# wangronin/Bayesian-Optimization

Hardware: AMD Instinct MI355X
Metric: candidates/sec (GP posterior+EI) at N=2048,d=20 and ask() wall-time, 1/2/4/8 GPU (higher is better)
Workload: dtype f64

## Files before the change

### bayesian-optimization_amd/_lib.py

```python
from __future__ import annotations

import ctypes as C
import functools
import os
from typing import Optional, Sequence, Tuple

import numpy as np

HERE = os.path.dirname(os.path.abspath(__file__))
LIB_PATH = os.path.join(HERE, "libbogp.so")

OK = 0
ERR_INVALID, ERR_HIP, ERR_NOT_POSDEF, ERR_UNSUPPORTED, ERR_NO_DEVICE, ERR_LLF_POSITIVE = -1, -2, -3, -4, -5, -6
KERNEL_SE, KERNEL_MATERN12, KERNEL_MATERN32, KERNEL_MATERN52, KERNEL_ABSEXP, KERNEL_CUBIC, KERNEL_GENEXP, KERNEL_MATERN_NU = 0, 1, 2, 3, 4, 5, 6, 7
MODE_NOISELESS, MODE_NOISY, MODE_NOISE_ESTIM = 0, 1, 2
ACQ_EI, ACQ_EPSILON_PI, ACQ_UCB, ACQ_MGFI = 0, 1, 2, 3
TREND_CONSTANT, TREND_LINEAR, TREND_QUADRATIC = 0, 1, 2
SELFTEST_PROFILE, SELFTEST_BESSEL_K, SELFTEST_RGAMMA, SELFTEST_BESSEL_K_PAIRS, SELFTEST_MATERN_NU_PAIRS = range(5)
ABI_VERSION = 9
MAX_Q = 64
PRUNE_PATH_NONE, PRUNE_PATH_CHUNKS, PRUNE_PATH_ONEPASS, PRUNE_PATH_ONEPASS_FALLBACK = 0, 1, 2, 3
MAX_TARGETS = 8
MAX_TOPK = 32
MAX_BELIEVED = 32
MAX_PATHS, MAX_FEATURES = 16, 16384
LIFT_MAX_R, LIFT_MAX_RD = 64, 4096
MAX_EHVI_CELLS = 65536
COMM_ID_BYTES = 128
COLUMN_REAL, COLUMN_DISCRETE = 0, 1
SCALES = {"linear": 0, None: 0, "log": 1, "log10": 2, "logit": 3, "bilog": 4}

_dp = C.POINTER(C.c_double)
_ip = C.POINTER(C.c_int)
_lp = C.POINTER(C.c_int64)

SIGNATURES = {
    "bogp_create": (C.c_int, [C.c_int, C.POINTER(C.c_void_p)]),
    "bogp_destroy": (None, [C.c_void_p]),
    "bogp_last_error": (C.c_char_p, [C.c_void_p]),
    "bogp_abi_version": (C.c_int, []),
    "bogp_set_train": (C.c_int, [C.c_void_p, _dp, _dp, C.c_int, C.c_int, C.c_int]),
    "bogp_select_target": (C.c_int, [C.c_void_p, C.c_int]),
    "bogp_nll": (C.c_int, [C.c_void_p, C.c_int, C.c_int, _dp, C.c_int, C.c_double, C.c_int, C.c_int, C.c_double, _dp, _dp]),
    "bogp_nll_batch": (C.c_int, [C.c_void_p, C.c_int, C.c_int, C.c_int, _dp, C.c_int, C.c_double, C.c_int, C.c_int, C.c_double, _dp, _dp, _ip]),
# ... 49 lines not shown
    "bogp_hessian": (C.c_int, [C.c_void_p, _dp, _dp]),
    "bogp_prior_corr": (C.c_int, [C.c_void_p, _dp, C.c_int, _dp]),
    "bogp_point_eval": (C.c_int, [C.c_void_p, _dp, C.c_int, _ip, _dp, C.c_double, C.c_int, _dp, _dp, _dp, _dp, _dp]),
    "bogp_point_eval_batch": (C.c_int, [C.c_void_p, _dp, C.c_int, C.c_int, _ip, _dp, C.c_double, C.c_int, _dp, _dp, _dp, _dp, _dp, _dp]),
    "bogp_polish": (C.c_int, [C.c_void_p, _dp, C.c_int, _dp, _dp, C.c_int, C.c_double, C.c_double, C.c_int, C.c_int, C.c_double,
                              C.c_double, _dp, _dp, _ip]),
    "bogp_point_eval_ehvi": (C.c_int, [C.c_void_p, _dp, C.c_int, C.c_int, C.c_int, _dp, _dp, _dp, _dp, _dp, _dp, _dp, _dp]),
    "bogp_polish_ehvi": (C.c_int, [C.c_void_p, _dp, C.c_int, _dp, _dp, C.c_int, C.c_int, _dp, _dp, C.c_int, C.c_double, C.c_double,
                                   _dp, _dp, _ip]),
    "bogp_comm_unique_id": (C.c_int, [C.c_char_p]),
    "bogp_comm_init": (C.c_int, [C.c_void_p, C.c_char_p, C.c_int, C.c_int]),
    "bogp_comm_attach": (C.c_int, [C.c_void_p, C.c_void_p]),
    "bogp_comm_info": (C.c_int, [C.c_void_p, _ip, _ip]),
    "bogp_comm_destroy": (C.c_int, [C.c_void_p]),
    "bogp_exchange_argmax": (C.c_int, [C.c_void_p, C.c_int64, _dp, _lp, _dp]),
    "bogp_exchange_topk": (C.c_int, [C.c_void_p, C.c_int64, _dp, _lp, _dp]),
    "bogp_reduce_pairs": (C.c_int, [C.c_int, C.c_int, C.c_int, _dp, _dp, _lp, _dp]),
    "bogp_merge_topk": (C.c_int, [C.c_int, C.c_int, C.c_int, C.c_int, _dp, _dp, _lp, _dp]),
    "bogp_last_timing": (C.c_int, [C.c_void_p, _dp, _dp, _dp, _ip]),
    "bogp_set_prune": (C.c_int, [C.c_void_p, C.c_int]),
    "bogp_last_contracted_rows": (C.c_int, [C.c_void_p, _lp]),
    "bogp_last_prune_path": (C.c_int, [C.c_void_p, _ip, _lp, _ip]),
    "bogp_prune_decide": (C.c_int, [C.c_int64, C.c_int64, C.c_int64, C.c_int64]),
    "bogp_sweep_chunk_rows": (C.c_int64, [C.c_int64, C.c_int64, C.c_int64]),
    "bogp_acq_upper_bound": (C.c_double, [C.c_int, C.c_double, C.c_double, C.c_double, C.c_double, C.c_double]),
    "bogp_prune_below": (C.c_int, [C.c_double, C.c_double]),
    "bogp_set_prune_bound32": (C.c_int, [C.c_void_p, C.c_int]),
    "bogp_last_bound32": (C.c_int, [C.c_void_p, _lp, _lp, _ip]),
    "bogp_debug_bound32": (C.c_int, [C.c_void_p, C.c_int64, _dp, _dp, _dp, _dp, C.POINTER(C.c_ubyte), _lp]),
    "bogp_debug_live": (None, [_lp, _lp, _lp]),
    "bogp_bound32_margin": (C.c_int, [C.c_int, C.c_int, C.c_double, C.c_double, C.c_double, C.c_double, _dp, _dp]),
    "bogp_acq_upper_bound_interval": (C.c_double, [C.c_int, C.c_double, C.c_double, C.c_double, C.c_double, C.c_double, C.c_double]),
    "bogp_flops_per_candidate": (C.c_double, [C.c_void_p]),
    "bogp_nll_path": (C.c_int, [C.c_int, C.c_int, C.c_int, C.c_int]),
    "bogp_chol_wide_panels": (C.c_int, [C.c_int, _ip, C.c_int]),
    "bogp_selftest_profile": (C.c_int, [C.c_void_p, C.c_int, C.c_int, C.c_double, _dp, C.c_int64, _dp]),
    "bogp_selftest_gemm": (C.c_int, [C.c_void_p, C.c_int, C.c_int, C.c_int, C.c_int, C.c_int, C.c_double, _dp, C.c_int, _dp, C.c_int, C.c_double, _dp, C.c_int, C.c_int, C.c_int]),
}

_lib = None


class BogpError(RuntimeError):
    def __init__(self, code: int, msg: str):
        super().__init__("libbogp error %d: %s" % (code, msg))
        self.code = code
# ... 888 lines not shown

    def last_bound32(self):
        rows, kept, fb = C.c_int64(), C.c_int64(), C.c_int()
        self._check(self._lib.bogp_last_bound32(self._h, C.cast(C.byref(rows), _lp), C.cast(C.byref(kept), _lp), C.cast(C.byref(fb), _ip)))
        return int(rows.value), int(kept.value), int(fb.value)

    def debug_bound32(self):
        n = C.c_int64()
        self._check(self._lib.bogp_debug_bound32(self._h, 0, None, None, None, None, None, C.cast(C.byref(n), _lp)))
        n = int(n.value)
        out = [np.empty(n) for _ in range(4)]
        flags = np.empty(n, dtype=np.uint8)
        if n:
            m = C.c_int64()
            self._check(self._lib.bogp_debug_bound32(self._h, n, _ptr(out[0]), _ptr(out[1]), _ptr(out[2]), _ptr(out[3]),
                                                     flags.ctypes.data_as(C.POINTER(C.c_ubyte)), C.cast(C.byref(m), _lp)))
        return out[0], out[1], out[2], out[3], flags

    def last_contracted_rows(self) -> int:
        n = C.c_int64()
        self._check(self._lib.bogp_last_contracted_rows(self._h, C.cast(C.byref(n), _lp)))
        return int(n.value)

    def selftest_gemm(self, A, B, C_in=None, ta=False, tb=False, alpha=1.0, beta=0.0, tri=0, split=True):
        A = np.asfortranarray(A, dtype=np.float64)
        B = np.asfortranarray(B, dtype=np.float64)
        m, k = (A.shape[1], A.shape[0]) if ta else A.shape
        k2, n = (B.shape[1], B.shape[0]) if tb else B.shape
        if k != k2:
            raise ValueError("inner dimensions differ: %d vs %d" % (k, k2))
        out = np.zeros((m, n), order="F") if C_in is None else np.asfortranarray(C_in, dtype=np.float64).copy(order="F")
        self._check(self._lib.bogp_selftest_gemm(self._h, int(ta), int(tb), m, n, k, float(alpha), _ptr(A), A.shape[0], _ptr(B), B.shape[0],
                                                 float(beta), _ptr(out), out.shape[0], int(tri), int(split)))
        return out

    def flops_per_candidate(self) -> float:
        return float(self._lib.bogp_flops_per_candidate(self._h))

    def selftest_profile(self, what, arg, kernel=0, pexp=0.0):
        arg = np.ascontiguousarray(arg, dtype=np.float64)
        n = arg.shape[0] if what >= SELFTEST_BESSEL_K_PAIRS else arg.size
        if what >= SELFTEST_BESSEL_K_PAIRS and (arg.ndim != 2 or arg.shape[1] != 2):
            raise ValueError("the *_PAIRS selectors take an (n, 2) array")
        out = np.empty(n)
        self._check(self._lib.bogp_selftest_profile(self._h, int(what), int(kernel), float(pexp), _ptr(arg), n, _ptr(out)))
        return out
# ... 1 lines not shown
```

### bayesian-optimization_amd/csrc/bogp_api.hip

```cpp
#include <hip/hip_runtime.h>

#include <algorithm>
#include <atomic>
#include <cmath>
#include <cstdio>
#include <cstdlib>
#include <cstring>
#include <string>
#include <vector>

#include "../../include/bogp.h"
#include "bogp_handle.h"
#include "bogp_internal.h"
#include "bogp_fit.h"

using namespace bogp;

static std::string g_create_error;

extern "C" int bogp_abi_version(void) { return BOGP_ABI_VERSION; }

extern "C" const char* bogp_last_error(const bogp_handle* h) { return h ? h->err.c_str() : g_create_error.c_str(); }

extern "C" int bogp_create(int device, bogp_handle** out) {
// ... 1 lines not shown
  *out = nullptr;
  int ndev = 0;
  hipError_t e = hipGetDeviceCount(&ndev);
  if (e != hipSuccess || ndev <= 0) {
    g_create_error = std::string("no HIP device: ") + hipGetErrorString(e);
    return BOGP_ERR_NO_DEVICE;
  }
  if (device < 0 || device >= ndev) {
    g_create_error = "device index out of range";
    return BOGP_ERR_INVALID;
  }
  hipDeviceProp_t prop;
  if (hipGetDeviceProperties(&prop, device) != hipSuccess) {
    g_create_error = "hipGetDeviceProperties failed";
    return BOGP_ERR_HIP;
  }
  if (strncmp(prop.gcnArchName, "gfx950", 6) != 0) {
    g_create_error = std::string("libbogp is built for gfx950 only; device is ") + prop.gcnArchName;
    return BOGP_ERR_NO_DEVICE;
  }
  bogp_handle* h = new bogp_handle();
  h->device = device;
  h->n_cu = prop.multiProcessorCount > 0 ? prop.multiProcessorCount : 256;
  int prio_least = 0, prio_greatest = 0;
  if (hipSetDevice(device) != hipSuccess || hipDeviceGetStreamPriorityRange(&prio_least, &prio_greatest) != hipSuccess ||
      hipStreamCreateWithPriority(&h->stream, hipStreamNonBlocking, prio_greatest) != hipSuccess ||
      hipStreamCreateWithPriority(&h->stream2, hipStreamNonBlocking, prio_least) != hipSuccess ||
      h->dscal.ensure(h, 64) != BOGP_OK) {
    g_create_error = "stream creation failed";
    delete h;
    return BOGP_ERR_HIP;
  }
  if (h->hfit.ensure(h, 4096) != BOGP_OK) {
    g_create_error = "pinned host buffer allocation failed";
    delete h;
    return BOGP_ERR_HIP;
  }
  h->hfit_dev = h->hfit.dev;
  if (h->dfin_ticket.ensure(h, 1) != BOGP_OK || hipMemset(h->dfin_ticket, 0, sizeof(unsigned int)) != hipSuccess) {
    g_create_error = "device allocation failed";
    delete h;
    return BOGP_ERR_HIP;
  }
  h->dinfo = reinterpret_cast<int*>(h->dscal + 62);
  if (!h->ev_chol.at(1)) {
    g_create_error = "event creation failed";
// ... 245 lines not shown
```

### bayesian-optimization_amd/csrc/bogp_api_sweep.hip

```cpp
#include <hip/hip_runtime.h>

#include <algorithm>
#include <atomic>
#include <cmath>
#include <cstdio>
#include <cstdlib>
#include <cstring>
#include <string>
#include <vector>

#include "../../include/bogp.h"
#include "bogp_device.h"
#include "bogp_handle.h"
#include "bogp_internal.h"
#include "bogp_fit.h"

using namespace bogp;

void bogp::invalidate_sweep_results(bogp_handle* h) { h->last_q = h->last_topk_q = h->last_topk_k = 0; }

static int lazy_copy_to(bogp_handle* h, int64_t upto) {
  if (!h->hXs_lazy) return BOGP_OK;
  upto = std::min<int64_t>(upto, h->M);
  if (upto <= h->lazy_done) return BOGP_OK;
// ... 542 lines not shown
      aa.uu = h->duu;
    }
  }
  aa.mtrend = h->dmtrend;
  aa.estimate_trend = 0;
  return BOGP_OK;
}

static int sweep_pruned_chunk(bogp_handle* h, SweepCtx& cx, const AcqArgs& model, const ContractArgs& ka, int64_t c, int64_t c_end, int64_t m0, int64_t mcount, int64_t skip) {
  hipStream_t st = cx.st;
  long long* const pctl = cx.pctl;
  const int64_t Mc = cx.g.Mc, Ms = cx.Ms, nblk_total = cx.nblk_total;
  const int q = cx.rq.q;
  hipEvent_t* ev = &h->ev[(size_t)(c * EPC)];
  int64_t i0 = 0;
  if (skip > 0) i0 = skip;
  else if (c == 0) {
    const int64_t P = std::min<int64_t>(PRUNE_PILOT, mcount);
    hipEvent_t* evp = &h->ev[(size_t)(cx.g.nchunk * EPC + 1)];
    HIPCHK(h, launch_prune_init(pctl, h->dbest_val, h->dbest_idx, q, P, st));
    HIPCHK(h, hipEventRecord(evp[0], st));
    ContractArgs kp = ka;
    kp.nMt = (int)((P + 63) / 64);
    HIPCHK(h, launch_contract(kp, st));
    HIPCHK(h, hipEventRecord(evp[1], st));
    AcqArgs ap = model;
    ap.mu_part = h->dmu_part[0]; ap.w_part = h->dw_part[0]; ap.ss_part = h->dss_part; ap.Mc = Mc; ap.mcount = P; ap.m0 = 0;
    HIPCHK(h, launch_acquisition(ap, st));
    HIPCHK(h, launch_prune_update(h->dblk_val, h->dblk_idx, nblk_total, nullptr, P, q, h->dbest_val, h->dbest_idx, st));
    i0 = P;
  }
  const int64_t rcount = mcount - i0;
  if (rcount > 0) {
    PruneBoundArgs pb = prune_bound_args(h, cx);
    pb.mu_part = h->dmu_part[0] + i0; pb.w_part = h->dw_part[0] + i0; pb.Mc = Mc; pb.rcount = rcount;
    HIPCHK(h, launch_prune_bound(pb, st));
    HIPCHK(h, launch_prune_scan(cx.pblk_count, (rcount + 255) / 256, cx.poffsets, rcount, Ms, pctl, st));
    PruneGatherArgs pg;
    pg.ctl = pctl; pg.flags = cx.pflags; pg.offsets = cx.poffsets; pg.rcount = rcount; pg.m0 = m0 + i0; pg.Mc = Mc; pg.Ms = Ms; pg.S = cx.g.S;
    pg.Np = h->Np; pg.rT = h->drT[0] + i0; pg.mu_part = h->dmu_part[0] + i0; pg.w_part = h->dw_part[0] + i0;
    pg.rTs = h->drT[1]; pg.mu_s = h->dmu_part[1]; pg.w_s = h->dw_part[1]; pg.sel = cx.psel; pg.map = cx.pmap;
    HIPCHK(h, launch_prune_gather(pg, st));
    cx.prune_pending += rcount / 4;
  }
  const bool flush = cx.prune_pending > 0 && (c + 1 == c_end || cx.prune_pending + Mc / 4 > Ms);
  HIPCHK(h, hipEventRecord(ev[2], st));
  if (rcount > 0) {
    ContractArgs ki = ka;
    ki.rT = h->drT[0] + i0; ki.ss_part = h->dss_part + i0; ki.nMt = (int)((rcount + 63) / 64); ki.live = pctl + 1;
    HIPCHK(h, launch_contract(ki, st));
  }
  if (flush) {
    ContractArgs kf = ka;
    kf.rT = h->drT[1]; kf.ss_part = cx.dss_surv; kf.Mc = Ms; kf.nMt = (int)(Ms / 64); kf.live = pctl + 0;
    HIPCHK(h, launch_contract(kf, st));
  }
  HIPCHK(h, hipEventRecord(ev[3], st));
  if (rcount > 0) {
    AcqArgs ai = model;
    ai.mu_part = h->dmu_part[0] + i0; ai.w_part = h->dw_part[0] + i0; ai.ss_part = h->dss_part + i0; ai.Mc = Mc; ai.mcount = rcount;
    ai.m0 = m0 + i0; ai.live = pctl + 1;
    HIPCHK(h, launch_acquisition(ai, st));
    HIPCHK(h, launch_prune_update(h->dblk_val, h->dblk_idx, nblk_total, pctl + 1, 0, q, h->dbest_val, h->dbest_idx, st));
  }
  if (flush) {
    AcqArgs af = model;
    af.mu_part = h->dmu_part[1]; af.w_part = h->dw_part[1]; af.ss_part = cx.dss_surv; af.Mc = Ms; af.mcount = Ms; af.m0 = 0;
    af.live = pctl + 0; af.map = cx.pmap;
    HIPCHK(h, launch_acquisition(af, st));
    HIPCHK(h, launch_prune_update(h->dblk_val, h->dblk_idx, nblk_total, pctl + 0, 0, q, h->dbest_val, h->dbest_idx, st));
    HIPCHK(h, launch_prune_flushed(pctl, st));
    cx.prune_pending = 0;
  }
  HIPCHK(h, hipEventRecord(ev[4], st));
  return BOGP_OK;
}

static int sweep_chunks(bogp_handle* h, SweepCtx& cx, int64_t c_begin, int64_t c_end, bool pilot_done) {
// ... 17 lines not shown
    ka.rT = h->drT[b]; ka.Vp = vx ? h->dVpx : h->dVp; ka.ss_part = h->dss_part; ka.Mc = Mc; ka.nMt = (int)(Mc_eff / 64); ka.nJ = cx.nJ;
    ka.NJ16 = cx.NJ16; ka.NKP = cx.Nrows / 8;
    if (overlap && c >= 2) HIPCHK(h, hipStreamWaitEvent(stP, h->ev[(size_t)((c - 2) * EPC + 4)], 0));
    if (overlap && vx && c >= 1) HIPCHK(h, hipStreamWaitEvent(stP, h->ev[(size_t)((c - 1) * EPC + 4)], 0));
    int e;
    if ((e = lazy_copy_to(h, m0 + mcount)) || (e = lazy_wait(h, stP)) || (stP != st && (e = lazy_wait(h, st)))) return e;
    HIPCHK(h, hipEventRecord(ev[0], stP));
    const int64_t skip = pilot_done && c == 0 ? std::min<int64_t>(PRUNE_PILOT, mcount) : 0;
    if (skip > 0) {
      ca.m0 += skip; ca.rT += skip; ca.mu_part += skip; ca.w_part += skip;
    }
    if (Mc_eff > skip) HIPCHK(h, launch_corr_chunk(h->kernel, ca, (int)((Mc_eff - skip) / 64), S, stP));
    if (vx) {
      if (h->vx_Ne > Np) HIPCHK(h, hipMemsetAsync(h->drT[b] + (size_t)Np * Mc, 0, (size_t)(h->vx_Ne - Np) * Mc * sizeof(double), stP));
      HIPCHK(h, launch_trend_rows(h->trend, h->dXs, m0, mcount, Mc_eff, h->d, Mc, h->dbetav, h->drT[b] + (size_t)h->vx_Ne * Mc, h->p,
                                  h->vx_Nt - h->vx_Ne, h->dmtrend, stP));
    }
    HIPCHK(h, hipEventRecord(ev[1], stP));
    if (overlap) HIPCHK(h, hipStreamWaitEvent(st, ev[1], 0));
    if (cx.prune) {
      if ((e = sweep_pruned_chunk(h, cx, model, ka, c, c_end, m0, mcount, skip))) return e;
    } else {
      HIPCHK(h, hipEventRecord(ev[2], st));
      if (rq.need_var) HIPCHK(h, launch_contract(ka, st));
      HIPCHK(h, hipEventRecord(ev[3], st));
      AcqArgs aa = model;
      aa.mu_part = h->dmu_part[b]; aa.w_part = h->dw_part[b]; aa.ss_part = h->dss_part; aa.nJ = rq.need_var ? cx.nJ_main : 0; aa.Mc = Mc;
      aa.nJ_plus = vx ? cx.nJ - cx.nJ_main : 0;
      aa.mcount = mcount; aa.m0 = m0; aa.blk_offset = cx.blk_offset;
      if (h->p > 1 && (e = sweep_trend_chunk(h, cx, b, m0, mcount, Mc_eff, aa))) return e;
      if (rq.eh) {
        EhviArgs ea = *rq.eh;
        ea.rT = h->drT[b]; ea.ss_part = h->dss_part; ea.w_part = h->dw_part[b]; ea.S = S; ea.nJ = cx.nJ_main; ea.Mc = Mc;
        ea.mcount = mcount; ea.m0 = m0; ea.beta = h->beta; ea.G = h->G; ea.estimate_trend = h->estimate_trend;
        ea.ehvi_out = h->dacq_out; ea.mu_out = rq.want_out ? h->dmu_out : nullptr; ea.mse_out = rq.want_out ? h->dmse_out : nullptr;
        ea.blk_val = h->dblk_val; ea.blk_idx = h->dblk_idx; ea.blk_offset = cx.blk_offset;
        HIPCHK(h, launch_ehvi(ea, st));
      } else {
        HIPCHK(h, launch_acquisition(aa, st));
      }
      HIPCHK(h, hipEventRecord(ev[4], st));
    }
    cx.blk_offset += (mcount + 255) / 256;
    if ((e = lazy_copy_to(h, m0 + mcount + Mc))) return e;
  }
  return BOGP_OK;
}
// ... 23 lines not shown
  const int64_t P = std::min<int64_t>(PRUNE_PILOT, Mc);
  long long* const hcount = reinterpret_cast<long long*>(h->hfit + 3504);
  size_t ev_next = (size_t)(nchunk * EPC + 3);
  h->t_spans.clear(); h->t_chunks.clear();
  int e;
  auto survivors_of = [&](int64_t rows, int64_t index_from, long long* out, const unsigned char* flags, int64_t* sidx, const int64_t* through) -> int {
    HIPCHK(h, launch_prune_scan(cx.pblk_count, (rows + 255) / 256, cx.poffsets, rows, -1, pctl, st));
    if (index_from >= 0) HIPCHK(h, launch_prune_index(flags, cx.poffsets, rows, index_from, cx.sidx_cap, sidx, st, through));
    HIPCHK(h, hipMemcpyAsync(hcount, pctl + PRUNE_CTL_TOTAL, sizeof(long long), hipMemcpyDeviceToHost, st));
    HIPCHK(h, hipStreamSynchronize(st));
    *out = *hcount;
    return BOGP_OK;
  };
  const CorrArgs cc = corr_chunk_args(h, cx.g, 0, 1);
  ContractArgs kc;
  kc.rT = h->drT[1]; kc.Vp = h->dVp; kc.ss_part = cx.dss_surv; kc.Mc = Ms; kc.nJ = cx.nJ; kc.NJ16 = cx.NJ16; kc.NKP = cx.Nrows / 8;
  AcqArgs aa = acq_model_args(h, cx.rq, S, cx.nJ_main, nblk_total);
  aa.mu_part = h->dmu_part[1]; aa.w_part = h->dw_part[1]; aa.ss_part = cx.dss_surv; aa.Mc = Ms; aa.m0 = 0;
  PruneBoundArgs pb = prune_bound_args(h, cx);
  Bound32Model md32{h->dX32, h->dvec32, h->dvec32 + h->Np, h->dvec32 + 2 * (size_t)h->Np, h->stats32[0], h->stats32[1], h->stats32[2]};
  int contract_launches = 0;
  auto evaluate = [&](int64_t cnt, const int64_t* map) -> int {
    kc.nMt = (int)((cnt + 63) / 64);
    if (int e2 = timed_span(h, st, &ev_next, 1, [&] { return launch_contract(kc, st); })) return e2;
    ++contract_launches;
    aa.mcount = cnt; aa.map = map;
    HIPCHK(h, launch_acquisition(aa, st));
    HIPCHK(h, launch_prune_update(h->dblk_val, h->dblk_idx, nblk_total, nullptr, cnt, q, h->dbest_val, h->dbest_idx, st));
    return BOGP_OK;
  };
  auto fall_back = [&](int64_t c0, int64_t c1, int path) -> int {
    int e2;
    if ((e2 = h->drT[0].ensure(h, (size_t)cx.Nrows * Mc))) return e2;
    if ((e2 = sweep_chunks(h, cx, c0, c1, true))) return e2;
    for (int64_t c = c0; c < c1; ++c) h->t_chunks.push_back(c);
    contract_launches += (int)(c1 - c0);
    h->prune_path = path;
    return BOGP_OK;
  };
  if ((e = mark_event(h, st, &ev_next, &h->t_total[0]))) return e;
  HIPCHK(h, launch_prune_init(pctl, h->dbest_val, h->dbest_idx, q, P, st));
  if ((e = timed_span(h, st, &ev_next, 0, [&] { return launch_corr_chunk(kernel, cc, (int)(P / 64), S, st); }))) return e;
  if ((e = evaluate(P, nullptr))) return e;
  long long pilot_surv = 0;
  pb.mu_part = h->dmu_part[1]; pb.w_part = h->dw_part[1]; pb.Mc = Ms; pb.rcount = P;
  HIPCHK(h, launch_prune_bound(pb, st));
  if ((e = survivors_of(P, -1, &pilot_surv, cx.pflags, cx.psidx, nullptr))) return e;
// ... 270 lines not shown
  if (rounds) *rounds = h->prune_rounds;
  return BOGP_OK;
}

extern "C" int bogp_prune_decide(int64_t pilot_rows, int64_t pilot_survivors, int64_t segment_rows, int64_t segment_survivors) {
  return prune_decide(pilot_rows, pilot_survivors, segment_rows, segment_survivors);
}
extern "C" int64_t bogp_sweep_chunk_rows(int64_t rows, int64_t M, int64_t chunk_bytes) { return sweep_chunk_rows(rows, M, chunk_bytes); }

extern "C" int bogp_last_contracted_rows(bogp_handle* h, int64_t* rows) {
  if (!h) return BOGP_ERR_INVALID;
  if (!rows) FAIL(h, BOGP_ERR_INVALID, "bogp_last_contracted_rows: null output");
  *rows = h->contracted_rows;
  if (h->prune_used && h->dprune) {
    HIPCHK(h, hipSetDevice(h->device));
    long long n = 0;
    HIPCHK(h, hipMemcpyAsync(&n, h->dprune + PRUNE_CTL_CONTRACTED, sizeof(n), hipMemcpyDeviceToHost, h->stream));
    HIPCHK(h, hipStreamSynchronize(h->stream));
    *rows = (int64_t)n + h->prune_survivors;
  }
  return BOGP_OK;
}

extern "C" double bogp_acq_upper_bound(int acq_id, double acq_par, double y_hat, double sd_ub, double plugin, double sigma2) {
  return acq_upper_bound(acq_id, acq_par, y_hat, sd_ub, plugin, sigma2);
}
extern "C" int bogp_prune_below(double bound, double threshold) { return prune_below(bound, threshold) ? 1 : 0; }

extern "C" double bogp_flops_per_candidate(const bogp_handle* h) {
  if (!h || !h->committed) return 0.0;
  const double N = h->N, d = h->d, p = h->estimate_trend ? 1 : 0;
  return N * N + N * (3 * d + 5 + 2 * p);
}

extern "C" int bogp_gradient(bogp_handle* h, const double* x, double* dmu, double* dmse) {
  if (!h) return BOGP_ERR_INVALID;
  if (!h->committed) FAIL(h, BOGP_ERR_INVALID, "bogp_gradient: no committed model");
  if (h->kernel == BOGP_KERNEL_CUBIC || h->kernel == BOGP_KERNEL_GENEXP || h->kernel == BOGP_KERNEL_MATERN_NU) FAIL(h, BOGP_ERR_UNSUPPORTED, "bogp_gradient: the cubic correlation has no input-derivative (corr_dx leaves it undefined in the reference, gpr.py:655-658)");
  if (!x || !dmu || !dmse) FAIL(h, BOGP_ERR_INVALID, "bogp_gradient: null pointer");
  const int N = h->N, d = h->d;
  hipStream_t st = h->stream;
  HIPCHK(h, hipSetDevice(h->device));
  const int pt = h->p;
  if (pt == 1)
    return point_eval_host(h, "bogp_gradient", x, 1, 0, nullptr, nullptr, 0.0, 1, nullptr, nullptr, dmu, dmse, nullptr, nullptr);
  if (pt > 1 && h->trend == BOGP_TREND_QUADRATIC)
// ... 139 lines not shown
```

### bayesian-optimization_amd/csrc/bogp_handle.h

```cpp
#pragma once
#include <hip/hip_runtime.h>

#include <atomic>
#include <cstdio>
#include <cstring>
#include <string>
#include <vector>

#include "../../include/bogp.h"
#include "bogp_internal.h"

struct bogp_handle;
namespace bogp {
void comm_release(bogp_handle* h);
std::vector<bogp_handle*> nll_team(bogp_handle* h, int P);
int point_eval_host(bogp_handle* h, const char* who, const double* Xb, int B, int q, const int* acq_id, const double* acq_par,
                    double plugin, int minimize, double* mu, double* mse, double* dmu, double* dmse, double* acq, double* dacq);
struct SweepRequest {
  bool want_out = false, want_acq_out = false;
  bool need_var = true, sync = true;
  int q = 0, minimize = 1;
  const int* acq_id = nullptr;
  const double* acq_par = nullptr;
  double plugin = 0.0;
// ... 113 lines not shown
  int kernel = 0, mode = 0, estimate_trend = 0;
  double beta = 0, G = 0, sigma2 = 0, noise_var = 0, llf = 0, ftft = 0;
  bogp::DevBuf<double> dXthT;
  bogp::DevBuf<double> dXnorm;
  bogp::DevBuf<double2> dVpx;
  bogp::DevBuf<double> dAtx;
  int vx_Ne = 0, vx_Nt = 0;
  bogp::DevBuf<double2> dVp;

  const double* dXs = nullptr;
  bogp::DevBuf<double> dXs_owned;
  bogp::DevBuf<double> dbounds;
  bogp::DevBuf<double> dxform;
  std::vector<double> h_xform;
  bogp::DevBuf<double> dsobol;
  int64_t M = 0;
  const double* hXs_lazy = nullptr;
  int64_t lazy_done = 0;
  hipStream_t stream_copy = nullptr;
  bogp::EventPool ev_copy{hipEventDisableTiming};

  bogp::DevBuf<double> drT[2], dmu_part[2], dw_part[2];
  bogp::DevBuf<double> dss_part;
  bogp::DevBuf<double> dblk_val, dmu_out, dmse_out, dacq_out, dbest_val;
  bogp::DevBuf<int64_t> dblk_idx, dbest_idx;
  bogp::DevBuf<unsigned int> dcounter;
  int prune_mode = 1;
  int prune_path = 0;
  int64_t prune_survivors = 0;
  int prune_rounds = 0;
  bogp::DevBuf<long long> dprune;
  int prune_bound32 = 1;
  bogp::DevBuf<float> dX32, dvec32;
  bogp::DevBuf<double> dstats32;
  double stats32[3] = {0, 0, 0};
  uint64_t commit_gen = 0, b32_gen = 0;
  int b32_target = -1;
  int64_t b32_rows = 0, b32_kept = 0;
  int b32_fallbacks = 0;
  size_t b32_ws_row32 = 0, b32_ws_flag1 = 0, b32_ws_rmax = 0;
  int64_t b32_last_rows = 0;
  bool prune_used = false;
  int64_t contracted_rows = 0;
  bogp::DevBuf<double> dtopk_val;
  bogp::DevBuf<int64_t> dtopk_idx;
  bogp::DevBuf<double> dehvi_cells;
// ... 148 lines not shown
```

### bayesian-optimization_amd/csrc/bogp_internal.h

```cpp
#pragma once
#include <hip/hip_runtime.h>
#include <stdint.h>

#include <string>

#include "../../include/bogp.h"

namespace bogp {

struct CorrArgs {
  const double* Xs;
  int64_t M;
  int64_t m0;
  int64_t Mc;
  int d;
  int Np;
  int nblk_per_split;
  const double* sqrt_theta;
  const double* XthT;
  const double* xnorm = nullptr;
  const double* gamma;
  const double* wvec;
  double* rT;
  bool store = true;
// ... 7 lines not shown
inline int train_ld(int N) { return N > 3072 ? ((N + 127) / 128) * 128 : ((N + 63) / 64) * 64; }
constexpr int SWEEP_NBLK_PER_SPLIT = 8;
inline int sweep_slices(int Np) { return (Np / 32 + SWEEP_NBLK_PER_SPLIT - 1) / SWEEP_NBLK_PER_SPLIT; }
constexpr int64_t SWEEP_MAX_CHUNK_ROWS = ((((int64_t)1 << 29) - 31) / 7) / 64 * 64;
inline int64_t sweep_chunk_rows(int64_t rows, int64_t M, int64_t chunk_bytes) {
  const int64_t Mpad = (M + 63) / 64 * 64, fit = chunk_bytes / (rows * (int64_t)sizeof(double)) / 64 * 64;
  const int64_t Mc = fit < 64 ? 64 : fit < Mpad ? fit : Mpad;
  return Mc > SWEEP_MAX_CHUNK_ROWS ? -1 : Mc;
}
int corr_trend_columns(int p);
bool corr_chunk_without_store(int kernel, int pv, bool have_xnorm);

struct ContractArgs {
  const double* rT;
  const double2* Vp;
  double* ss_part;
  int64_t Mc;
  int nMt;
  int nJ;
  int NJ16;
  int NKP;
  int64_t cross_B;
  const long long* live = nullptr;
};

struct AcqArgs {
  const double* mu_part;
  const double* w_part;
  const double* ss_part;
  int S, nJ;
  int nJ_plus = 0;
  int64_t Mc;
  int64_t mcount;
  int64_t m0;
  double beta;
  const double* mtrend;
  const double* uu;
  double G;
  int estimate_trend;
  double sigma2;
  double* mu_out;
  double* mse_out;
  int q;
  int acq_id[64];
  double acq_par[64];
  double plugin;
// ... 249 lines not shown
  double beta, G, sigma2, plugin;
  int estimate_trend, minimize, q;
  int acq_id[64];
  double acq_par[64];
  double* mu_out;
  double* mse_out;
  double* acq_out;
  double* blk_val;
  int64_t* blk_idx;
  int64_t nblk;
  unsigned int* counter;
  double* best_val;
  int64_t* best_idx;
  long long* stamps;
  int64_t m_begin;
  int64_t blk_begin;
  int final_launch;
};
bool sweep_small_supported(int Np, int d, int kernel);
int64_t sweep_small_blocks(int64_t M, int n_cu);
hipError_t launch_sweep_small(int kernel, const SmallArgs& a, int n_cu, hipStream_t st);

hipError_t launch_corr_chunk(int kernel, const CorrArgs& a, int nMt, int S, hipStream_t st);
hipError_t launch_contract(const ContractArgs& a, hipStream_t st);
hipError_t launch_contract_cross(const ContractArgs& a, int ncp, hipStream_t st);
int contract_cols_per_group();
hipError_t launch_acquisition(const AcqArgs& a, hipStream_t st);
hipError_t launch_argmax_final(const double* blk_val, const int64_t* blk_idx, int64_t nblk, int64_t stride, int q,
                               double* out_val, int64_t* out_idx, hipStream_t st);

hipError_t launch_topk(const double* vals, int64_t M, int q, int k, double* blk_val, int64_t* blk_idx, double* out_val,
                       int64_t* out_idx, hipStream_t st);

struct LiftArgs {
  const double* Z;
  int64_t M;
  int r, D;
  const double* lift;
  double* penalty;
  int* blk_count;
};
size_t lift_lds_bytes(int r, int D);
hipError_t launch_lift_penalty(const LiftArgs& a, hipStream_t st);
hipError_t launch_lift_scan(const int* blk_count, int64_t nblk, int64_t* offsets, hipStream_t st);
hipError_t launch_lift_compact(const double* Z, int64_t M, int r, const double* penalty, const int64_t* offsets, double* Zc,
                               int64_t* map, hipStream_t st);
hipError_t launch_lift_merge(const double* penalty, int64_t M, const double* acq, const int64_t* map, int64_t Mf, int q,
// ... 236 lines not shown
```

### bayesian-optimization_amd/csrc/kernels_posterior.hip

```cpp
#include <algorithm>
#include <cstdlib>

#include "bogp_device.h"
#include "bogp_internal.h"
#include "bogp_mfma.h"

namespace bogp {

struct CorrDims {
  int64_t M, m0, Mc;
  int d, Np, nblk_per_split;
  int wld;
};
template <int KERNEL, int PV>
__global__ __launch_bounds__(256) void k_corr_chunk(const double* __restrict__ Xs, const double* __restrict__ sqrt_theta,
                                                    const double* __restrict__ XthT, const double* __restrict__ gamma,
                                                    const double* __restrict__ wvec, double* __restrict__ rT,
                                                    double* __restrict__ mu_part, double* __restrict__ w_part,
                                                    const double* __restrict__ Wrow, double* __restrict__ t_part, CorrDims a) {
  extern __shared__ __attribute__((aligned(16))) double smem[];
  double* xs = smem;
  const int tid = threadIdx.x;
  const int m = tid & 63;
  const int g = __builtin_amdgcn_readfirstlane(tid >> 6);
// ... 87 lines not shown
                                                   CorrDims a) {
#define BOGP_CORR_STORE 1
#include "corr_mfma_body.inc"
#undef BOGP_CORR_STORE
}
template <int KERNEL>
__global__ __launch_bounds__(256) __attribute__((amdgpu_waves_per_eu(4, 4))) void k_corr_mfma_sums(const double* __restrict__ Xs, const double* __restrict__ sqrt_theta,
                                                   const double* __restrict__ XthT, const double* __restrict__ xnorm,
                                                   const double* __restrict__ gamma, const double* __restrict__ wvec,
                                                   double* __restrict__ mu_part, double* __restrict__ w_part, CorrDims a) {
#define BOGP_CORR_STORE 0
#include "corr_mfma_body.inc"
#undef BOGP_CORR_STORE
}

#undef BOGP_OPQ
constexpr int MR = 4;
constexpr int NWJ = 4;
constexpr int KB = 32;
constexpr int PITCH = 64 + 16;



template <int NR>
__device__ __forceinline__ void contract_drain(d4 (&acc)[MR][NR]) {
#ifndef BOGP_LINT_NO_DRAIN
  mfma16_drain();
#endif
#ifndef BOGP_LINT_NO_FENCE
#pragma unroll
  for (int mi = 0; mi < MR; ++mi)
#pragma unroll
    for (int ni = 0; ni < NR; ++ni) mfma16_fence(acc[mi][ni]);
#endif
}

template <int NR, bool GUARDED>
__device__ __forceinline__ void contract_block16(const double* __restrict__ tile, const double2* __restrict__ vp,
                                                 const size_t (&boff)[NR], const int (&jt)[NR], int aoff, int kb, int kp_last,
                                                 double2 (&bq)[4][NR], d4 (&acc)[MR][NR]) {
  double af[2][MR];
#pragma unroll
  for (int mi = 0; mi < MR; ++mi) af[0][mi] = tile[aoff + 16 * mi];
#pragma unroll
  for (int s = 0; s < 4; ++s) {
    const int kp = kb * 4 + s;
    const int kb16 = kp >> 1;
    {
      const int kpn = min(kp + 2, kp_last);
#pragma unroll
      for (int ni = 0; ni < NR; ++ni) bq[(s + 2) & 3][ni] = vp[boff[ni] + (size_t)kpn * 64];
    }
#pragma unroll
    for (int h = 0; h < 2; ++h) {
// ... 322 lines not shown
    red2[w * 64 + lane] = s;
  }
  BOGP_DT_NOW(5);
  __syncthreads();
  if (tid < 64) {
    const double tot = ((red2[tid] + red2[64 + tid]) + red2[128 + tid]) + red2[192 + tid];
    a.ss_part[(size_t)jg * a.Mc + mc0 + tid] = tot;
  }
#ifdef CONTRACT_D_TRACE
  BOGP_DT_NOW(6);
  dtr[7] = (unsigned long long)nkp | ((unsigned long long)nkp_full << 32);
  __syncthreads();
  if (trace_out) {
    unsigned long long* dst = trace_out + (size_t)blockIdx.x * (NWJ * DT_NST);
    const unsigned long long* src = &dtr_all[0][0];
    for (int i = tid; i < NWJ * DT_NST; i += 256) dst[i] = src[i];
  }
#endif
}
#undef BOGP_DT_NOW
#undef BOGP_DT_ISSUE
#undef BOGP_DT_STORE

static bool corr_sqdist_kernel(int kernel) {
  return kernel == BOGP_KERNEL_SE || kernel == BOGP_KERNEL_MATERN12 || kernel == BOGP_KERNEL_MATERN32 || kernel == BOGP_KERNEL_MATERN52;
}
bool corr_chunk_without_store(int kernel, int pv, bool have_xnorm) { return corr_sqdist_kernel(kernel) && pv == 0 && have_xnorm; }

hipError_t launch_corr_chunk(int kernel, const CorrArgs& a, int nMt, int S, hipStream_t st) {
  dim3 grid((unsigned)nMt, (unsigned)S);
  if (corr_chunk_without_store(kernel, a.pv, a.xnorm != nullptr)) {
    const int KS = (a.d + 3) / 4;
    const size_t shm = (size_t)max(4 * KS * 64, 2048) * sizeof(double);
    CorrDims dm{a.M, a.m0, a.Mc, a.d, a.Np, a.nblk_per_split, a.wld};
#define BOGP_LAUNCH_CORR_MFMA(K)                                                                                                      \
  do {                                                                                                                                \
    if (shm > 64 * 1024) {                                                                                                            \
      hipError_t e_ = hipFuncSetAttribute(reinterpret_cast<const void*>(&k_corr_mfma<K>), hipFuncAttributeMaxDynamicSharedMemorySize, \
                                          (int)shm);                                                                                  \
      if (e_ != hipSuccess) return e_;                                                                                                \
    }                                                                                                                                 \
    hipLaunchKernelGGL((k_corr_mfma<K>), grid, 256, shm, st, a.Xs, a.sqrt_theta, a.XthT, a.xnorm, a.gamma, a.wvec, a.rT, a.mu_part,   \
                       a.w_part, dm);                                                                                                 \
  } while (0)
#define BOGP_LAUNCH_CORR_SUMS(K)                                                                                                      \
  do {                                                                                                                                \
// ... 63 lines not shown

#ifdef CONTRACT_D_TRACE
static unsigned long long* g_trace = nullptr;
static size_t g_trace_words = 0, g_trace_used = 0;
static int g_trace_dims[4] = {0, 0, 0, 0};
hipError_t debug_contract_trace(unsigned long long* out, size_t cap_words, size_t* used_words, int* dims) {
  if (used_words) *used_words = g_trace_used;
  if (dims) for (int i = 0; i < 4; ++i) dims[i] = g_trace_dims[i];
  if (!out) return hipSuccess;
  hipError_t e = hipDeviceSynchronize();
  if (e != hipSuccess) return e;
  return hipMemcpy(out, g_trace, std::min(cap_words, g_trace_used) * sizeof(unsigned long long), hipMemcpyDeviceToHost);
}
#else
static bool contract_direct() {
  static const bool on = [] {
    const char* e = getenv("BOGP_CONTRACT_DIRECT");
    return !(e && atoi(e) == 0);
  }();
  return on;
}
#endif

hipError_t launch_contract(const ContractArgs& a, hipStream_t st) {
  const dim3 grid((unsigned)(a.nMt * a.nJ));
#ifdef CONTRACT_D_TRACE
  const size_t need = (size_t)a.nMt * a.nJ * NWJ * DT_NST;
  if (need > g_trace_words) {
    if (g_trace) (void)hipFree(g_trace);
    hipError_t e = hipMalloc((void**)&g_trace, need * sizeof(unsigned long long));
    if (e != hipSuccess) return e;
    g_trace_words = need;
  }
  const bool keep = need >= g_trace_used;
  if (keep) {
    g_trace_used = need;
    g_trace_dims[0] = a.nMt; g_trace_dims[1] = a.nJ; g_trace_dims[2] = a.NJ16; g_trace_dims[3] = DT_NST;
  }
  hipLaunchKernelGGL(k_contract16d, grid, 256, 0, st, a, keep ? g_trace : (unsigned long long*)nullptr);
#else
  if (contract_direct()) hipLaunchKernelGGL(k_contract16d, grid, 256, 0, st, a);
  else hipLaunchKernelGGL(k_contract16<4>, grid, 256, 0, st, a);
#endif
  return hipGetLastError();
}

int contract_cols_per_group() { return NWJ * 4 * 16; }

hipError_t launch_contract_cross(const ContractArgs& a, int ncp, hipStream_t st) {
  const dim3 grid((unsigned)(a.nMt * a.nJ));
  if (ncp == 16) hipLaunchKernelGGL((k_contract16<4, 16>), grid, 256, 0, st, a);
  else if (ncp == 32) hipLaunchKernelGGL((k_contract16<4, 32>), grid, 256, 0, st, a);
  else if (ncp == 64) hipLaunchKernelGGL((k_contract16<4, 64>), grid, 256, 0, st, a);
  else return hipErrorInvalidValue;
  return hipGetLastError();
}

}
```

### include/bogp.h

```cpp
#ifndef BOGP_H
#define BOGP_H

#include <stdint.h>

#ifdef __cplusplus
extern "C" {
#endif

typedef struct bogp_handle bogp_handle;

#define BOGP_ABI_VERSION 9
#define BOGP_OK 0
#define BOGP_ERR_INVALID (-1)
#define BOGP_ERR_HIP (-2)
#define BOGP_ERR_NOT_POSDEF (-3)
#define BOGP_ERR_UNSUPPORTED (-4)
#define BOGP_ERR_NO_DEVICE (-5)
#define BOGP_ERR_LLF_POSITIVE (-6)

#define BOGP_KERNEL_SE 0
#define BOGP_KERNEL_MATERN12 1
#define BOGP_KERNEL_MATERN32 2
#define BOGP_KERNEL_MATERN52 3
#define BOGP_KERNEL_ABSEXP 4
// ... 156 lines not shown
int bogp_comm_info(const bogp_handle* h, int* rank, int* world);
int bogp_comm_destroy(bogp_handle* h);
int bogp_exchange_argmax(bogp_handle* h, int64_t index_offset, double* best_val, int64_t* best_gidx, double* best_x);
int bogp_exchange_topk(bogp_handle* h, int64_t index_offset, double* best_val, int64_t* best_gidx, double* best_x);
int bogp_reduce_pairs(int R, int q, int d, const double* gathered, double* val, int64_t* gidx, double* x);
int bogp_merge_topk(int R, int q, int k, int d, const double* gathered, double* val, int64_t* gidx, double* x);

int bogp_last_timing(bogp_handle* h, double* corr_ms, double* contract_ms, double* acquisition_ms, int* n_chunks);

int bogp_set_prune(bogp_handle* h, int on);

#define BOGP_PRUNE_PATH_NONE 0
#define BOGP_PRUNE_PATH_CHUNKS 1
#define BOGP_PRUNE_PATH_ONEPASS 2
#define BOGP_PRUNE_PATH_ONEPASS_FALLBACK 3
int bogp_last_prune_path(bogp_handle* h, int* path, int64_t* survivors, int* rounds);

int bogp_prune_decide(int64_t pilot_rows, int64_t pilot_survivors, int64_t segment_rows, int64_t segment_survivors);

int64_t bogp_sweep_chunk_rows(int64_t rows, int64_t M, int64_t chunk_bytes);

int bogp_last_contracted_rows(bogp_handle* h, int64_t* rows);

double bogp_acq_upper_bound(int acq_id, double acq_par, double y_hat, double sd_ub, double plugin, double sigma2);
int bogp_prune_below(double bound, double threshold);

int bogp_set_prune_bound32(bogp_handle* h, int on);

int bogp_last_bound32(bogp_handle* h, int64_t* rows, int64_t* kept, int* fallbacks);

int bogp_debug_bound32(bogp_handle* h, int64_t cap, double* mu32, double* e_mu, double* wd32, double* e_w, unsigned char* flags, int64_t* rows);

void bogp_debug_live(int64_t* allocations, int64_t* bytes, int64_t* events);

int bogp_bound32_margin(int kernel, int d, double na, double nb_max, double gamma_l1, double w_l1, double* e_mu, double* e_w);
double bogp_acq_upper_bound_interval(int acq_id, double acq_par, double y_hat, double e, double sd_ub, double plugin, double sigma2);

double bogp_flops_per_candidate(const bogp_handle* h);

int bogp_selftest_gemm(bogp_handle* h, int ta, int tb, int m, int n, int k, double alpha, const double* A, int lda,
                       const double* B, int ldb, double beta, double* C, int ldc, int tri, int split);

#define BOGP_SELFTEST_PROFILE 0
#define BOGP_SELFTEST_BESSEL_K 1
#define BOGP_SELFTEST_RGAMMA 2
#define BOGP_SELFTEST_BESSEL_K_PAIRS 3
// ... 19 lines not shown
```

Measured before the change: 531.8 million.

## Add smaller-row contract kernels chosen by occupancy heuristic for small candidate batches

```diff
diff --git a/bayesian-optimization_amd/_lib.py b/bayesian-optimization_amd/_lib.py
--- a/bayesian-optimization_amd/_lib.py
+++ b/bayesian-optimization_amd/_lib.py
@@ -20,6 +20,7 @@
 ABI_VERSION = 9
 MAX_Q = 64
 PRUNE_PATH_NONE, PRUNE_PATH_CHUNKS, PRUNE_PATH_ONEPASS, PRUNE_PATH_ONEPASS_FALLBACK = 0, 1, 2, 3
+CONTRACT_TILE64_MIN_WG_PER_4CU, CONTRACT_TILE32_MIN_WG_PER_4CU = 14, 6
 MAX_TARGETS = 8
 MAX_TOPK = 32
 MAX_BELIEVED = 32
@@ -115,6 +116,9 @@
     "bogp_last_contracted_rows": (C.c_int, [C.c_void_p, _lp]),
     "bogp_last_prune_path": (C.c_int, [C.c_void_p, _ip, _lp, _ip]),
     "bogp_prune_decide": (C.c_int, [C.c_int64, C.c_int64, C.c_int64, C.c_int64]),
+    "bogp_set_contract_tile": (C.c_int, [C.c_void_p, C.c_int]),
+    "bogp_last_contract_tile": (C.c_int, [C.c_void_p, _ip]),
+    "bogp_contract_tile_rows": (C.c_int, [C.c_int64, C.c_int, C.c_int, C.c_int]),
     "bogp_sweep_chunk_rows": (C.c_int64, [C.c_int64, C.c_int64, C.c_int64]),
     "bogp_acq_upper_bound": (C.c_double, [C.c_int, C.c_double, C.c_double, C.c_double, C.c_double, C.c_double]),
     "bogp_prune_below": (C.c_int, [C.c_double, C.c_double]),
@@ -1049,6 +1053,16 @@
         self._check(self._lib.bogp_last_contracted_rows(self._h, C.cast(C.byref(n), _lp)))
         return int(n.value)
 
+    def set_contract_tile(self, rows=0):
+        if rows not in (0, 16, 32, 64):
+            raise ValueError("set_contract_tile: %r is none of 0 (automatic), 16, 32, 64" % (rows,))
+        self._check(self._lib.bogp_set_contract_tile(self._h, int(rows)))
+
+    def last_contract_tile(self) -> int:
+        n = C.c_int()
+        self._check(self._lib.bogp_last_contract_tile(self._h, C.cast(C.byref(n), _ip)))
+        return int(n.value)
+
     def selftest_gemm(self, A, B, C_in=None, ta=False, tb=False, alpha=1.0, beta=0.0, tri=0, split=True):
         A = np.asfortranarray(A, dtype=np.float64)
         B = np.asfortranarray(B, dtype=np.float64)
diff --git a/bayesian-optimization_amd/csrc/bogp_api.hip b/bayesian-optimization_amd/csrc/bogp_api.hip
--- a/bayesian-optimization_amd/csrc/bogp_api.hip
+++ b/bayesian-optimization_amd/csrc/bogp_api.hip
@@ -47,6 +47,7 @@
   bogp_handle* h = new bogp_handle();
   h->device = device;
   h->n_cu = prop.multiProcessorCount > 0 ? prop.multiProcessorCount : 256;
+  h->contract_tile.n_cu = h->n_cu;
   int prio_least = 0, prio_greatest = 0;
   if (hipSetDevice(device) != hipSuccess || hipDeviceGetStreamPriorityRange(&prio_least, &prio_greatest) != hipSuccess ||
       hipStreamCreateWithPriority(&h->stream, hipStreamNonBlocking, prio_greatest) != hipSuccess ||
diff --git a/bayesian-optimization_amd/csrc/bogp_api_sweep.hip b/bayesian-optimization_amd/csrc/bogp_api_sweep.hip
--- a/bayesian-optimization_amd/csrc/bogp_api_sweep.hip
+++ b/bayesian-optimization_amd/csrc/bogp_api_sweep.hip
@@ -588,7 +588,7 @@
     HIPCHK(h, hipEventRecord(evp[0], st));
     ContractArgs kp = ka;
     kp.nMt = (int)((P + 63) / 64);
-    HIPCHK(h, launch_contract(kp, st));
+    HIPCHK(h, launch_contract(kp, st, h->contract_tile));
     HIPCHK(h, hipEventRecord(evp[1], st));
     AcqArgs ap = model;
     ap.mu_part = h->dmu_part[0]; ap.w_part = h->dw_part[0]; ap.ss_part = h->dss_part; ap.Mc = Mc; ap.mcount = P; ap.m0 = 0;
@@ -614,12 +614,12 @@
   if (rcount > 0) {
     ContractArgs ki = ka;
     ki.rT = h->drT[0] + i0; ki.ss_part = h->dss_part + i0; ki.nMt = (int)((rcount + 63) / 64); ki.live = pctl + 1;
-    HIPCHK(h, launch_contract(ki, st));
+    HIPCHK(h, launch_contract(ki, st, h->contract_tile));
   }
   if (flush) {
     ContractArgs kf = ka;
     kf.rT = h->drT[1]; kf.ss_part = cx.dss_surv; kf.Mc = Ms; kf.nMt = (int)(Ms / 64); kf.live = pctl + 0;
-    HIPCHK(h, launch_contract(kf, st));
+    HIPCHK(h, launch_contract(kf, st, h->contract_tile));
   }
   HIPCHK(h, hipEventRecord(ev[3], st));
   if (rcount > 0) {
@@ -683,7 +683,7 @@
       if ((e = sweep_pruned_chunk(h, cx, model, ka, c, c_end, m0, mcount, skip))) return e;
     } else {
       HIPCHK(h, hipEventRecord(ev[2], st));
-      if (rq.need_var) HIPCHK(h, launch_contract(ka, st));
+      if (rq.need_var) HIPCHK(h, launch_contract(ka, st, h->contract_tile));
       HIPCHK(h, hipEventRecord(ev[3], st));
       AcqArgs aa = model;
       aa.mu_part = h->dmu_part[b]; aa.w_part = h->dw_part[b]; aa.ss_part = h->dss_part; aa.nJ = rq.need_var ? cx.nJ_main : 0; aa.Mc = Mc;
@@ -753,7 +753,7 @@
   int contract_launches = 0;
   auto evaluate = [&](int64_t cnt, const int64_t* map) -> int {
     kc.nMt = (int)((cnt + 63) / 64);
-    if (int e2 = timed_span(h, st, &ev_next, 1, [&] { return launch_contract(kc, st); })) return e2;
+    if (int e2 = timed_span(h, st, &ev_next, 1, [&] { return launch_contract(kc, st, h->contract_tile); })) return e2;
     ++contract_launches;
     aa.mcount = cnt; aa.map = map;
     HIPCHK(h, launch_acquisition(aa, st));
@@ -1070,6 +1070,20 @@
   return BOGP_OK;
 }
 
+extern "C" int bogp_set_contract_tile(bogp_handle* h, int rows) {
+  if (!h) return BOGP_ERR_INVALID;
+  if (rows != 0 && rows != 16 && rows != 32 && rows != 64) FAIL(h, BOGP_ERR_INVALID, "bogp_set_contract_tile: %d is none of 0 (automatic), 16, 32, 64", rows);
+  h->contract_tile.forced = rows;
+  return BOGP_OK;
+}
+extern "C" int bogp_last_contract_tile(bogp_handle* h, int* rows) {
+  if (!h) return BOGP_ERR_INVALID;
+  if (!rows) FAIL(h, BOGP_ERR_INVALID, "bogp_last_contract_tile: null output");
+  *rows = h->contract_tile.last;
+  return BOGP_OK;
+}
+extern "C" int bogp_contract_tile_rows(int64_t row_tiles64, int nJ, int n_cu, int live) { return contract_tile_rows(row_tiles64, nJ, n_cu, live != 0); }
+
 extern "C" double bogp_acq_upper_bound(int acq_id, double acq_par, double y_hat, double sd_ub, double plugin, double sigma2) {
   return acq_upper_bound(acq_id, acq_par, y_hat, sd_ub, plugin, sigma2);
 }
diff --git a/bayesian-optimization_amd/csrc/bogp_handle.h b/bayesian-optimization_amd/csrc/bogp_handle.h
--- a/bayesian-optimization_amd/csrc/bogp_handle.h
+++ b/bayesian-optimization_amd/csrc/bogp_handle.h
@@ -159,6 +159,7 @@
 
   bogp::DevBuf<double> drT[2], dmu_part[2], dw_part[2];
   bogp::DevBuf<double> dss_part;
+  bogp::ContractTile contract_tile;
   bogp::DevBuf<double> dblk_val, dmu_out, dmse_out, dacq_out, dbest_val;
   bogp::DevBuf<int64_t> dblk_idx, dbest_idx;
   bogp::DevBuf<unsigned int> dcounter;
diff --git a/bayesian-optimization_amd/csrc/bogp_internal.h b/bayesian-optimization_amd/csrc/bogp_internal.h
--- a/bayesian-optimization_amd/csrc/bogp_internal.h
+++ b/bayesian-optimization_amd/csrc/bogp_internal.h
@@ -53,6 +53,21 @@
   int NKP;
   int64_t cross_B;
   const long long* live = nullptr;
+};
+
+constexpr int CONTRACT_TILE64_MIN_WG_PER_4CU = 14;
+constexpr int CONTRACT_TILE32_MIN_WG_PER_4CU = 6;
+inline int contract_tile_rows(int64_t tiles64, int nJ, int n_cu, bool live) {
+  if (live) return 64;
+  const int64_t wg4 = 4 * tiles64 * (int64_t)(nJ > 0 ? nJ : 1), cu = n_cu > 0 ? n_cu : 1;
+  if (wg4 >= CONTRACT_TILE64_MIN_WG_PER_4CU * cu) return 64;
+  if (wg4 >= CONTRACT_TILE32_MIN_WG_PER_4CU * cu) return 32;
+  return 16;
+}
+struct ContractTile {
+  int n_cu = 0;
+  int forced = 0;
+  int last = 64;
 };
 
 struct AcqArgs {
@@ -348,7 +363,7 @@
 hipError_t launch_sweep_small(int kernel, const SmallArgs& a, int n_cu, hipStream_t st);
 
 hipError_t launch_corr_chunk(int kernel, const CorrArgs& a, int nMt, int S, hipStream_t st);
-hipError_t launch_contract(const ContractArgs& a, hipStream_t st);
+hipError_t launch_contract(const ContractArgs& a, hipStream_t st, ContractTile& ct);
 hipError_t launch_contract_cross(const ContractArgs& a, int ncp, hipStream_t st);
 int contract_cols_per_group();
 hipError_t launch_acquisition(const AcqArgs& a, hipStream_t st);
diff --git a/bayesian-optimization_amd/csrc/kernels_posterior.hip b/bayesian-optimization_amd/csrc/kernels_posterior.hip
--- a/bayesian-optimization_amd/csrc/kernels_posterior.hip
+++ b/bayesian-optimization_amd/csrc/kernels_posterior.hip
@@ -133,14 +133,14 @@
 
 
 
-template <int NR>
-__device__ __forceinline__ void contract_drain(d4 (&acc)[MR][NR]) {
+template <int MRT, int NR>
+__device__ __forceinline__ void contract_drain(d4 (&acc)[MRT][NR]) {
 #ifndef BOGP_LINT_NO_DRAIN
   mfma16_drain();
 #endif
 #ifndef BOGP_LINT_NO_FENCE
 #pragma unroll
-  for (int mi = 0; mi < MR; ++mi)
+  for (int mi = 0; mi < MRT; ++mi)
 #pragma unroll
     for (int ni = 0; ni < NR; ++ni) mfma16_fence(acc[mi][ni]);
 #endif
@@ -509,6 +509,139 @@
 #undef BOGP_DT_ISSUE
 #undef BOGP_DT_STORE
 
+template <int MRN> struct ContractAFrag;
+template <> struct ContractAFrag<1> { typedef double type; };
+template <> struct ContractAFrag<2> { typedef double2 type; };
+__device__ __forceinline__ double afrag_row(double a, int) { return a; }
+__device__ __forceinline__ double afrag_row(const double2& a, int mi) { return mi ? a.y : a.x; }
+
+template <int MRN, int DDN, int WPE>
+__global__ __launch_bounds__(256, WPE) void k_contract16n(ContractArgs a) {
+  constexpr int NR = 4;
+  constexpr int JT16 = NWJ * NR;
+  constexpr int ROWS = 16 * MRN;
+  constexpr int RP = ROWS + 1;
+  constexpr int DRN = DDN + 1;
+  typedef typename ContractAFrag<MRN>::type afrag;
+  __shared__ __attribute__((aligned(16))) double lds[16 * NWJ * RP + NWJ * ROWS];
+
+  const int tid = threadIdx.x;
+  const int lane = tid & 63;
+  const int w = __builtin_amdgcn_readfirstlane(tid >> 6);
+  const int nMt = a.nMt * (64 / ROWS);
+  const int jg = a.nJ - 1 - (int)(blockIdx.x / nMt);
+  const int mt = blockIdx.x % nMt;
+  const int64_t mc0 = (int64_t)mt * ROWS;
+  if (a.live && mc0 >= *a.live) return;
+  const int NJ16 = a.NJ16, NKP = a.NKP;
+  const int kmax16 = min((jg + 1) * JT16, NJ16);
+  const int nkp_full = 2 * jg * JT16;
+  const int nkp = min(2 * kmax16, max(2 * ((jg + 1) * JT16 - w), 2));
+  const int kp_last = nkp - 1;
+
+  int jt[NR];
+  bool valid[NR];
+  const char* vb[NR];
+#pragma unroll
+  for (int ni = 0; ni < NR; ++ni) {
+    const int j = jg * JT16 + ((ni & 1) ? NWJ * (ni + 1) - 1 - w : NWJ * ni + w);
+    valid[ni] = j < NJ16;
+    jt[ni] = valid[ni] ? j : -1;
+    vb[ni] = reinterpret_cast<const char*>(a.Vp + (size_t)min(j, NJ16 - 1) * NKP * 64);
+  }
+  const size_t Mc = (size_t)a.Mc;
+  const char* ab = reinterpret_cast<const char*>(a.rT + mc0);
+  const size_t kp_stride = 8 * Mc * sizeof(double);
+  unsigned voffA0 = (unsigned)(((size_t)(lane >> 4) * Mc + MRN * (lane & 15)) * sizeof(double));
+  unsigned voffA1 = voffA0 + (unsigned)(4 * Mc * sizeof(double));
+  unsigned voffB = (unsigned)lane * 16u;
+
+  d4 acc[MRN][NR];
+#pragma unroll
+  for (int mi = 0; mi < MRN; ++mi)
+#pragma unroll
+    for (int ni = 0; ni < NR; ++ni) acc[mi][ni] = (d4){0.0, 0.0, 0.0, 0.0};
+
+  afrag av[DRN][2];
+  double2 bv[DRN][NR];
+#define BOGP_N_LOAD1(slot, g, ap_, kpc_, vb_)                                                                         \
+  do {                                                                                                                \
+    if ((g) == 0) av[slot][0] = *reinterpret_cast<const afrag*>((ap_) + voffA0);                                      \
+    else if ((g) == 5) av[slot][1] = *reinterpret_cast<const afrag*>((ap_) + voffA1);                                 \
+    else bv[slot][(g) - 1] = ld2_plain((vb_)[(g) - 1] + (size_t)(kpc_) * 1024 + voffB);                               \
+  } while (0)
+#define BOGP_N_KPAIR(G, u, kp_)                                                                                       \
+  do {                                                                                                                \
+    const int kpc_ = min((kp_) + DDN, kp_last);                                                                       \
+    const char* ap_ = ab + (size_t)kpc_ * kp_stride;                                                                  \
+    const int k16_ = (kp_) >> 1;                                                                                      \
+    asm volatile("" : "+v"(voffA0), "+v"(voffA1), "+v"(voffB));                                                       \
+    const char* vbe_[NR];                                                                                             \
+    _Pragma("unroll") for (int ni = 0; ni < NR; ++ni) vbe_[ni] = (!(G) || ((kpc_ >> 1) <= jt[ni])) ? vb[ni] : vb[NR - 1]; \
+    _Pragma("unroll") for (int g = 0; g < 8; ++g) {                                                                   \
+      if (g == 0) {                                                                                                   \
+        _Pragma("unroll") for (int l_ = 0; l_ < 6; ++l_) BOGP_N_LOAD1(((u) + DDN) % DRN, l_, ap_, kpc_, vbe_);        \
+      }                                                                                                               \
+      __builtin_amdgcn_sched_barrier(0);                                                                              \
+      if (!(G) || k16_ <= jt[g & 3]) {                                                                                \
+        const double b_ = (g >> 2) == 0 ? bv[u][g & 3].x : bv[u][g & 3].y;                                            \
+        _Pragma("unroll") for (int mi = 0; mi < MRN; ++mi) mfma16(afrag_row(av[u][g >> 2], mi), b_, acc[mi][g & 3]);  \
+      }                                                                                                               \
+      __builtin_amdgcn_sched_barrier(0);                                                                              \
+    }                                                                                                                 \
+  } while (0)
+
+#pragma unroll
+  for (int t = 0; t < DDN; ++t) {
+    const int kpc = min(t, kp_last);
+    const char* ap = ab + (size_t)kpc * kp_stride;
+#pragma unroll
+    for (int g = 0; g < 6; ++g) BOGP_N_LOAD1(t, g, ap, kpc, vb);
+  }
+
+  int kp = 0;
+  for (; kp + DRN <= nkp_full; kp += DRN) {
+#pragma unroll
+    for (int u = 0; u < DRN; ++u) BOGP_N_KPAIR(false, u, kp + u);
+  }
+  for (; kp < nkp; kp += DRN) {
+#pragma unroll
+    for (int u = 0; u < DRN; ++u)
+      if (kp + u < nkp) BOGP_N_KPAIR(true, u, kp + u);
+  }
+#undef BOGP_N_KPAIR
+#undef BOGP_N_LOAD1
+
+  contract_drain(acc);
+  double* red = lds;
+  double* red2 = lds + 16 * NWJ * RP;
+  const int q = lane >> 4, jc = lane & 15;
+#pragma unroll
+  for (int mi = 0; mi < MRN; ++mi)
+#pragma unroll
+    for (int r = 0; r < 4; ++r) {
+      double s = 0.0;
+#pragma unroll
+      for (int ni = 0; ni < NR; ++ni)
+        if (valid[ni]) s = __builtin_fma(acc[mi][ni][r], acc[mi][ni][r], s);
+      red[(jc * NWJ + w) * RP + MRN * (4 * r + q) + mi] = s;
+    }
+  __builtin_amdgcn_fence(__ATOMIC_RELEASE, "workgroup");
+  __builtin_amdgcn_wave_barrier();
+  __builtin_amdgcn_fence(__ATOMIC_ACQUIRE, "workgroup");
+  if (lane < ROWS) {
+    double s = 0.0;
+#pragma unroll
+    for (int sl = 0; sl < 16; ++sl) s += red[(sl * NWJ + w) * RP + lane];
+    red2[w * ROWS + lane] = s;
+  }
+  __syncthreads();
+  if (tid < ROWS) {
+    const double tot = ((red2[tid] + red2[ROWS + tid]) + red2[2 * ROWS + tid]) + red2[3 * ROWS + tid];
+    a.ss_part[(size_t)jg * a.Mc + mc0 + tid] = tot;
+  }
+}
+
 static bool corr_sqdist_kernel(int kernel) {
   return kernel == BOGP_KERNEL_SE || kernel == BOGP_KERNEL_MATERN12 || kernel == BOGP_KERNEL_MATERN32 || kernel == BOGP_KERNEL_MATERN52;
 }
@@ -618,8 +751,12 @@
 }
 #endif
 
-hipError_t launch_contract(const ContractArgs& a, hipStream_t st) {
+constexpr int CONTRACT_DD32 = 4, CONTRACT_WPE32 = 2;
+constexpr int CONTRACT_DD16 = 4, CONTRACT_WPE16 = 3;
+
+hipError_t launch_contract(const ContractArgs& a, hipStream_t st, ContractTile& ct) {
   const dim3 grid((unsigned)(a.nMt * a.nJ));
+  ct.last = 64;
 #ifdef CONTRACT_D_TRACE
   const size_t need = (size_t)a.nMt * a.nJ * NWJ * DT_NST;
   if (need > g_trace_words) {
@@ -635,8 +772,16 @@
   }
   hipLaunchKernelGGL(k_contract16d, grid, 256, 0, st, a, keep ? g_trace : (unsigned long long*)nullptr);
 #else
-  if (contract_direct()) hipLaunchKernelGGL(k_contract16d, grid, 256, 0, st, a);
-  else hipLaunchKernelGGL(k_contract16<4>, grid, 256, 0, st, a);
+  if (!contract_direct()) {
+    hipLaunchKernelGGL(k_contract16<4>, grid, 256, 0, st, a);
+    return hipGetLastError();
+  }
+  const int rows = a.live ? 64 : ct.forced ? ct.forced : contract_tile_rows(a.nMt, a.nJ, ct.n_cu, false);
+  const dim3 gridn((unsigned)(a.nMt * (64 / rows) * a.nJ));
+  if (rows == 16) hipLaunchKernelGGL((k_contract16n<1, CONTRACT_DD16, CONTRACT_WPE16>), gridn, 256, 0, st, a);
+  else if (rows == 32) hipLaunchKernelGGL((k_contract16n<2, CONTRACT_DD32, CONTRACT_WPE32>), gridn, 256, 0, st, a);
+  else hipLaunchKernelGGL(k_contract16d, grid, 256, 0, st, a);
+  ct.last = rows;
 #endif
   return hipGetLastError();
 }
diff --git a/include/bogp.h b/include/bogp.h
--- a/include/bogp.h
+++ b/include/bogp.h
@@ -202,6 +202,11 @@
 
 int bogp_last_contracted_rows(bogp_handle* h, int64_t* rows);
 
+int bogp_set_contract_tile(bogp_handle* h, int rows);
+int bogp_last_contract_tile(bogp_handle* h, int* rows);
+
+int bogp_contract_tile_rows(int64_t row_tiles64, int nJ, int n_cu, int live);
+
 double bogp_acq_upper_bound(int acq_id, double acq_par, double y_hat, double sd_ub, double plugin, double sigma2);
 int bogp_prune_below(double bound, double threshold);
 
```

Result: faster. 603.4 million, median of 6 (+13.5%).
